# yangt1013/SPEINet

Hardware: AMD Instinct MI355X
Metric: deblurred 720p frames/sec (higher is better)
Workload: dtype f16 (correlation top2)

## Files before the change

### speinet_amd/csrc/conv64_ws16.hip

```cpp
#include "common.h"

namespace {

constexpr int C = 64, KS = 5, PAD = 2, NTAP = KS * KS;
constexpr int TH = 6, TW = 32;
constexpr int IH = TH + KS - 1, IW = TW + KS - 1;
constexpr int PITCH = 2 * C + 16;
constexpr int SLAB = IH * IW * PITCH;
constexpr int NTHR = 256;
constexpr int HR = TH / 2;
constexpr int XCH_WAVE = HR * 4 * 64 * 16;
constexpr int LDS_BYTES = 2 * SLAB + 4 * XCH_WAVE;
constexpr int PF = 1;

struct WsParams {
    const void* a;
    const void* wfrag;
    const float* bias;
    void* out;
    int H, W, batch, act;
    int tiles_x, tiles_y, total;
    long long* stamps;
};

__device__ __forceinline__ void mfma_aw(f32x16& acc, const lpv<_Float16>::x8& w, const lpv<_Float16>::x8& b) {
    asm volatile("v_mfma_f32_32x32x16_f16 %0, %1, %2, %0" : "+v"(acc) : "a"(w), "v"(b));
}
__device__ __forceinline__ void mfma_aw(f32x16& acc, const lpv<__bf16>::x8& w, const lpv<__bf16>::x8& b) {
    asm volatile("v_mfma_f32_32x32x16_bf16 %0, %1, %2, %0" : "+v"(acc) : "a"(w), "v"(b));
}
__device__ __forceinline__ void mfma_aw0(f32x16& acc, const lpv<_Float16>::x8& w, const lpv<_Float16>::x8& b) {
    asm volatile("v_mfma_f32_32x32x16_f16 %0, %1, %2, 0" : "=v"(acc) : "a"(w), "v"(b));
}
__device__ __forceinline__ void mfma_aw0(f32x16& acc, const lpv<__bf16>::x8& w, const lpv<__bf16>::x8& b) {
    asm volatile("v_mfma_f32_32x32x16_bf16 %0, %1, %2, 0" : "=v"(acc) : "a"(w), "v"(b));
}

template <typename TA> struct Chunk { static constexpr int CPP = sizeof(TA) == 4 ? 16 : 8; };

template <typename LP, typename TA, typename TO>
__global__ __launch_bounds__(NTHR, 1) void conv64_ws_kernel(const WsParams p) {
    typedef typename lpv<LP>::x8 lp8;
    typedef typename lpv<LP>::x4 lp4;
    constexpr int CPP = Chunk<TA>::CPP;
    constexpr int NCH = IH * IW * CPP;
    constexpr int NIT = (NCH + NTHR - 1) / NTHR;
    constexpr int NPH = sizeof(TA) == 4 ? 3 : 1;
    constexpr int NITH = (NIT + NPH - 1) / NPH;
    constexpr int PSTEP = 2 * NTAP / NPH;
    static_assert(NPH == 1 || NPH == 3, "the MFMA loop below is cut for one or three staging parts");
    extern __shared__ __attribute__((aligned(16))) unsigned char smem[];

    const int tid = threadIdx.x, lane = tid & 63, wave = tid >> 6;
    const int fr = lane & 31, fk = lane >> 5;
    const int nt = wave >> 1, kh = wave & 1;

    lp8 wreg[NTAP][2];
    {
        const LP* wp = static_cast<const LP*>(p.wfrag) + ((size_t)nt * NTAP * 4 + 2 * kh) * 512 + lane * 8;
#pragma unroll
        for (int t = 0; t < NTAP; ++t)
#pragma unroll
            for (int s = 0; s < 2; ++s) wreg[t][s] = *reinterpret_cast<const lp8*>(wp + (t * 4 + s) * 512);
    }
    float biasv[16];
#pragma unroll
    for (int r = 0; r < 16; ++r) biasv[r] = p.bias ? p.bias[32 * nt + 8 * (r >> 2) + 4 * fk + (r & 3)] : 0.f;

    typedef u32x4 stage_t;
    stage_t sreg[NITH];
    const size_t map_elems = (size_t)p.H * p.W * C;
    const int per_map = p.tiles_x * p.tiles_y;
    const int G = gridDim.x;
    const int slot = (G & 7) ? (int)blockIdx.x : (int)(blockIdx.x & 7) * (G >> 3) + (int)(blockIdx.x >> 3);
    auto tile_of = [&](int t) {
        const int base = t - (int)blockIdx.x;
        return base + G <= p.total ? base + slot : t;
    };
    auto tile_origin = [&](int t, int& b, int& oy0, int& ox0) {
        t = tile_of(t);
        b = t / per_map;
        const int r = t - b * per_map;
        const int ty = r / p.tiles_x;
        oy0 = ty * TH;
        ox0 = (r - ty * p.tiles_x) * TW;
    };
    constexpr int PPI = NTHR / CPP, E = 16 / (int)sizeof(TA);
    const int p0 = tid / CPP, sub = tid - p0 * CPP;
    const int iy0 = p0 / IW, ix0 = p0 - iy0 * IW;
    const int lds0 = p0 * PITCH + sub * (sizeof(TA) == 4 ? 8 : 16);
    auto advance = [](int& iy, int& ix) {
        ix += PPI % IW;
        iy += PPI / IW;
        if (ix >= IW) { ix -= IW; ++iy; }
    };
    auto load_slab = [&](int t, int ph) {
        int b, oy0, ox0;
        tile_origin(t, b, oy0, ox0);
        const TA* base = static_cast<const TA*>(p.a) + (size_t)b * map_elems + sub * E;
        int iy = iy0, ix = ix0;
#pragma unroll
        for (int it = 0; it < NIT; ++it) {
            if (it >= ph * NITH && it < (ph + 1) * NITH) {
                const int iyc = min(iy, IH - 1);
                const int gy = min(max(oy0 - PAD + iyc, 0), p.H - 1), gx = min(max(ox0 - PAD + ix, 0), p.W - 1);
                sreg[it - ph * NITH] = *reinterpret_cast<const stage_t*>(base + ((size_t)gy * p.W + gx) * C);
            }
            advance(iy, ix);
        }
    };
    auto store_slab = [&](int t, int buf, int ph, int lo, int hi) {
        int b, oy0, ox0;
        tile_origin(t, b, oy0, ox0);
        unsigned char* sl = smem + buf * SLAB + lds0;
        int iy = iy0, ix = ix0;
#pragma unroll
        for (int it = 0; it < NIT; ++it) {
            if (it >= ph * NITH + lo && it < ph * NITH + hi && it < (ph + 1) * NITH && iy < IH) {
                const int j = it - ph * NITH;
                const bool ok = ((unsigned)(oy0 - PAD + iy) < (unsigned)p.H) & ((unsigned)(ox0 - PAD + ix) < (unsigned)p.W);
                if constexpr (sizeof(TA) == 4) {
                    const f32x4 v = __builtin_bit_cast(f32x4, sreg[j]);
                    lp4 h = to_lp4<LP>(v);
                    if (!ok) h = lp4{(LP)0.f, (LP)0.f, (LP)0.f, (LP)0.f};
                    *reinterpret_cast<lp4*>(sl + it * PPI * PITCH) = h;
                } else {
                    *reinterpret_cast<stage_t*>(sl + it * PPI * PITCH) = ok ? sreg[j] : stage_t{0u, 0u, 0u, 0u};
                }
            }
            advance(iy, ix);
        }
    };

    int t = blockIdx.x;
    if (t >= p.total) return;
#pragma unroll
    for (int ph = 0; ph < NPH; ++ph) {
        load_slab(t, ph);
        store_slab(t, 0, ph, 0, NITH);
    }
    lds_barrier();

    int boff[TH];
#pragma unroll
    for (int i = 0; i < TH; ++i) boff[i] = (((i + HR * kh) % TH) * IW + fr) * PITCH + kh * 64 + fk * 16;
    unsigned char* const xch = smem + 2 * SLAB;

    int buf = 0;
    for (; t < p.total; t += gridDim.x, buf ^= 1) {
        const int tn = t + gridDim.x;
        const bool more = tn < p.total;
        const int tl = more ? tn : t;
        const bool st_ = t == (int)blockIdx.x + (int)gridDim.x;
        if (st_) SPEI_STAMP(p.stamps, 0);
        load_slab(tl, 0);
        if (st_) SPEI_STAMP(p.stamps, 1);
        __builtin_amdgcn_sched_barrier(0);

        const unsigned char* sl = smem + buf * SLAB;
        f32x16 acc[TH];
        lp8 bq[PF + 1][TH];
        auto step_off = [](int step) { const int tap = step >> 1; return ((tap / KS) * IW + (tap % KS)) * PITCH + (step & 1) * 32; };
#pragma unroll
        for (int d = 0; d < PF; ++d)
#pragma unroll
            for (int i = 0; i < TH; ++i) bq[d][i] = *reinterpret_cast<const lp8*>(sl + boff[i] + step_off(d));
        auto steps = [&](auto lo_c, auto hi_c) {
            constexpr int LO = decltype(lo_c)::value, HI = decltype(hi_c)::value;
#pragma unroll
            for (int step = LO; step < HI; ++step) {
                const int tap = step >> 1, s2 = step & 1;
                if (step + PF < NTAP * 2) {
#pragma unroll
                    for (int i = 0; i < TH; ++i)
                        bq[(step + PF) % (PF + 1)][i] = *reinterpret_cast<const lp8*>(sl + boff[i] + step_off(step + PF));
                }
#pragma unroll
                for (int i = 0; i < TH; ++i) {
                    if (step == 0) mfma_aw0(acc[i], wreg[tap][s2], bq[step % (PF + 1)][i]);
                    else mfma_aw(acc[i], wreg[tap][s2], bq[step % (PF + 1)][i]);
                }
                if (NPH == 1 && step >= NTAP && ((step - NTAP) & 1) == 0 && (step - NTAP) / 2 < NITH)
                    store_slab(tl, buf ^ 1, 0, (step - NTAP) / 2, (step - NTAP) / 2 + 1);
            }
        };
        if constexpr (NPH == 1) {
            steps(std::integral_constant<int, 0>{}, std::integral_constant<int, 2 * NTAP>{});
        } else {
            steps(std::integral_constant<int, 0>{}, std::integral_constant<int, PSTEP>{});
            store_slab(tl, buf ^ 1, 0, 0, NITH);
            load_slab(tl, 1);
            steps(std::integral_constant<int, PSTEP>{}, std::integral_constant<int, 2 * PSTEP>{});
            store_slab(tl, buf ^ 1, 1, 0, NITH);
            load_slab(tl, 2);
            steps(std::integral_constant<int, 2 * PSTEP>{}, std::integral_constant<int, 2 * NTAP>{});
        }

        __builtin_amdgcn_sched_barrier(0);
        asm volatile("s_nop 7\n\ts_nop 7\n\ts_nop 7" ::: "memory");
        __builtin_amdgcn_sched_barrier(0);
        if (st_) SPEI_STAMP(p.stamps, 2);
        {
            f32x4* x = reinterpret_cast<f32x4*>(xch + wave * XCH_WAVE) + lane;
#pragma unroll
            for (int j = 0; j < HR; ++j)
#pragma unroll
                for (int g = 0; g < 4; ++g)
                    x[(j * 4 + g) * 64] = f32x4{acc[HR + j][4 * g], acc[HR + j][4 * g + 1], acc[HR + j][4 * g + 2], acc[HR + j][4 * g + 3]};
        }
        lds_barrier();
        if (st_) SPEI_STAMP(p.stamps, 3);
        {
            int b, oy0, ox0;
            tile_origin(t, b, oy0, ox0);
            TO* ob = static_cast<TO*>(p.out) + (size_t)b * map_elems;
            const int ox = ox0 + fr;
            const f32x4* x = reinterpret_cast<const f32x4*>(xch + (wave ^ 1) * XCH_WAVE) + lane;
#pragma unroll
            for (int j = 0; j < HR; ++j) {
                const int oy = oy0 + kh * HR + j;
                if (oy < p.H && ox < p.W) {
                    TO* o = ob + ((size_t)oy * p.W + ox) * C + 32 * nt + 4 * fk;
#pragma unroll
                    for (int g = 0; g < 4; ++g) {
                        const f32x4 q = x[(j * 4 + g) * 64];
                        f32x4 v;
#pragma unroll
                        for (int e = 0; e < 4; ++e) {
                            v[e] = acc[j][4 * g + e] + q[e] + biasv[4 * g + e];
                            if (p.act == SPEI_ACT_RELU) v[e] = fmaxf(v[e], 0.f);
                        }
                        if constexpr (sizeof(TO) == 4) *reinterpret_cast<f32x4*>(o + 8 * g) = v;
                        else *reinterpret_cast<lp4*>(o + 8 * g) = to_lp4<LP>(v);
                    }
                }
            }
        }
        if (st_) SPEI_STAMP(p.stamps, 4);
        if (NPH > 1) store_slab(tl, buf ^ 1, NPH - 1, 0, NITH);
        else store_slab(tl, buf ^ 1, 0, (NTAP + 1) / 2, NITH);
        lds_barrier();
        if (st_) SPEI_STAMP(p.stamps, 5);
    }
}

template <typename LP>
int launch_ws(const WsParams& p, int a16, int o16, hipStream_t st) {
    const size_t lds = LDS_BYTES;
    const int cus = spei_num_cus();
    const dim3 grid(p.total < cus ? p.total : cus);
    if (a16 && o16) {
        ensure_dyn_lds<&conv64_ws_kernel<LP, LP, LP>>(lds);
        hipLaunchKernelGGL((conv64_ws_kernel<LP, LP, LP>), grid, dim3(NTHR), lds, st, p);
    } else if (!a16 && o16) {
        ensure_dyn_lds<&conv64_ws_kernel<LP, float, LP>>(lds);
        hipLaunchKernelGGL((conv64_ws_kernel<LP, float, LP>), grid, dim3(NTHR), lds, st, p);
    } else if (a16 && !o16) {
        ensure_dyn_lds<&conv64_ws_kernel<LP, LP, float>>(lds);
        hipLaunchKernelGGL((conv64_ws_kernel<LP, LP, float>), grid, dim3(NTHR), lds, st, p);
    } else {
        ensure_dyn_lds<&conv64_ws_kernel<LP, float, float>>(lds);
        hipLaunchKernelGGL((conv64_ws_kernel<LP, float, float>), grid, dim3(NTHR), lds, st, p);
    }
    return 0;
}

}

extern "C" int spei_conv64_ws16(int fmt, const void* a, int a_fmt, const void* wfrag, const float* bias, void* out, int out_fmt, int batch,
                                int H, int W, int act, spei_stream_t stream) {
    SPEI_REQUIRE(a && wfrag && out, "spei_conv64_ws16: null pointer");
    SPEI_REQUIRE((fmt == SPEI_BF16 || fmt == SPEI_F16) && (a_fmt == SPEI_F32 || a_fmt == fmt) && (out_fmt == SPEI_F32 || out_fmt == fmt),
                 "spei_conv64_ws16: fmt=%d a_fmt=%d out_fmt=%d", fmt, a_fmt, out_fmt);
    SPEI_REQUIRE(batch >= 1 && H > 0 && W > 0 && (int64_t)batch * cdiv(H, TH) * cdiv(W, TW) < (1ll << 30) && (int64_t)H * W < (1ll << 26),
                 "spei_conv64_ws16: batch=%d of %dx%d", batch, H, W);
    SPEI_REQUIRE(act == SPEI_ACT_NONE || act == SPEI_ACT_RELU, "spei_conv64_ws16: act=%d", act);
    SPEI_REQUIRE(((uintptr_t)a | (uintptr_t)wfrag | (uintptr_t)out) % 16 == 0 && a != out, "spei_conv64_ws16: 16-byte alignment, out must not be the input");
    WsParams p;
    p.a = a; p.wfrag = wfrag; p.bias = bias; p.out = out; p.H = H; p.W = W; p.batch = batch; p.act = act;
    p.tiles_x = cdiv(W, TW); p.tiles_y = cdiv(H, TH); p.total = batch * p.tiles_x * p.tiles_y;
    p.stamps = spei_stamp_buffer();
    hipStream_t st = (hipStream_t)stream;
    const int a16 = a_fmt != SPEI_F32, o16 = out_fmt != SPEI_F32;
    const int rc = fmt == SPEI_F16 ? launch_ws<_Float16>(p, a16, o16, st) : launch_ws<__bf16>(p, a16, o16, st);
    if (rc) return rc;
    SPEI_CHECK_LAUNCH("spei_conv64_ws16");
    return 0;
}
```

### speinet_amd/csrc/resblock.hip

```cpp
#include "common.h"

namespace {

constexpr int GATE_TR16 = 16;
constexpr int GATE_TR32 = 8;
__host__ __device__ inline int gate_tr(bool lp) { return lp ? GATE_TR16 : GATE_TR32; }
__host__ __device__ inline int gate_tc(int C) { return 256 / (C / 8); }

struct GateWs {
    float* rowpmax;
    float* rowpsum;
    float* colpmax;
    float* colpsum;
    float* tilesum;
    int ntx, nty;
};
__host__ __device__ inline GateWs carve(float* ws, int H, int W, int C, bool lp) {
    GateWs g;
    g.ntx = (W + gate_tc(C) - 1) / gate_tc(C);
    g.nty = (H + gate_tr(lp) - 1) / gate_tr(lp);
    g.rowpmax = ws;
    g.rowpsum = g.rowpmax + (size_t)g.ntx * H * C;
    g.colpmax = g.rowpsum + (size_t)g.ntx * H * C;
    g.colpsum = g.colpmax + (size_t)g.nty * W * C;
    g.tilesum = g.colpsum + (size_t)g.nty * W * C;
    return g;
}

template <typename T>
__device__ __forceinline__ f32x4 ld4(const T* p) {
    if constexpr (sizeof(T) == 4) {
        return *reinterpret_cast<const f32x4*>(p);
    } else {
        const typename lpv<T>::x4 h = *reinterpret_cast<const typename lpv<T>::x4*>(p);
        return f32x4{(float)h[0], (float)h[1], (float)h[2], (float)h[3]};
    }
}

__device__ __forceinline__ f32x4 max4(f32x4 a, f32x4 b) {
    return f32x4{fmaxf(a[0], b[0]), fmaxf(a[1], b[1]), fmaxf(a[2], b[2]), fmaxf(a[3], b[3])};
}

template <int C, typename TX>
__global__ __launch_bounds__(256) void gate_stats_kernel(const TX* __restrict__ x1, int H, int W, float* ws, int64_t wsf) {
    constexpr bool LP = sizeof(TX) == 2;
    x1 += (size_t)blockIdx.y * H * W * C;
    const GateWs g = carve(ws + (size_t)blockIdx.y * wsf, H, W, C, LP);
    constexpr int OCT = C / 8;
    constexpr int TC = 256 / OCT;
    constexpr int TR = LP ? GATE_TR16 : GATE_TR32;
    constexpr int EB = LP ? 16 : 32;
    constexpr int ROWB = TC * OCT * EB + 4 * EB;
    constexpr int ITEMS = TR * OCT;
    constexpr int PARTS = 256 / ITEMS;
    constexpr int SEG = TC / PARTS;
    extern __shared__ __attribute__((aligned(16))) unsigned char tile[];
    float* rsum = reinterpret_cast<float*>(tile + TR * ROWB);
    const int tid = threadIdx.x;
    const int oct = tid % OCT, col = tid / OCT;
    const int tx = blockIdx.x % g.ntx, ty = blockIdx.x / g.ntx;
    const int x = tx * TC + col, y0 = ty * TR;

    u32x4 v[TR][LP ? 1 : 2];
#pragma unroll
    for (int r = 0; r < TR; ++r) {
        const bool ok = x < W && y0 + r < H;
        const TX* src = x1 + ((size_t)min(y0 + r, H - 1) * W + min(x, W - 1)) * C + oct * 8;
#pragma unroll
        for (int hlf = 0; hlf < (LP ? 1 : 2); ++hlf) {
            v[r][hlf] = *reinterpret_cast<const u32x4*>(reinterpret_cast<const unsigned char*>(src) + 16 * hlf);
            if (!ok) v[r][hlf] = u32x4{0u, 0u, 0u, 0u};
        }
    }
    auto unpack = [](const u32x4* q, float* f) __attribute__((always_inline)) {
        if constexpr (LP) {
            const typename lpv<TX>::x8 h = *reinterpret_cast<const typename lpv<TX>::x8*>(q);
#pragma unroll
            for (int e = 0; e < 8; ++e) f[e] = (float)h[e];
        } else {
#pragma unroll
            for (int e = 0; e < 8; ++e) f[e] = __uint_as_float(q[e >> 2][e & 3]);
        }
    };
    float cmax[8], csum[8];
#pragma unroll
    for (int e = 0; e < 8; ++e) { cmax[e] = -INFINITY; csum[e] = 0.f; }
#pragma unroll
    for (int r = 0; r < TR; ++r) {
        float f[8];
        unpack(v[r], f);
        if (y0 + r < H) {
#pragma unroll
            for (int e = 0; e < 8; ++e) { cmax[e] = fmaxf(cmax[e], f[e]); csum[e] += f[e]; }
        }
#pragma unroll
        for (int hlf = 0; hlf < (LP ? 1 : 2); ++hlf)
            *reinterpret_cast<u32x4*>(tile + r * ROWB + (col * OCT + oct) * EB + 16 * hlf) = v[r][hlf];
    }
    if (x < W) {
        float* pm = g.colpmax + ((size_t)ty * W + x) * C + oct * 8;
        float* ps = g.colpsum + ((size_t)ty * W + x) * C + oct * 8;
        *reinterpret_cast<f32x4*>(pm) = f32x4{cmax[0], cmax[1], cmax[2], cmax[3]};
        *reinterpret_cast<f32x4*>(pm + 4) = f32x4{cmax[4], cmax[5], cmax[6], cmax[7]};
        *reinterpret_cast<f32x4*>(ps) = f32x4{csum[0], csum[1], csum[2], csum[3]};
        *reinterpret_cast<f32x4*>(ps + 4) = f32x4{csum[4], csum[5], csum[6], csum[7]};
    }
    __syncthreads();

    {
        const int part = tid % PARTS, item = tid / PARTS;
        const int ro = item % OCT, rr = item / OCT;
        float rmax[8], rs[8];
#pragma unroll
        for (int e = 0; e < 8; ++e) { rmax[e] = -INFINITY; rs[e] = 0.f; }
        const int ncol = min(TC, W - tx * TC);
#pragma unroll 4
        for (int j = 0; j < SEG; ++j) {
            const int c2 = j * PARTS + part;
            u32x4 q[LP ? 1 : 2];
#pragma unroll
            for (int hlf = 0; hlf < (LP ? 1 : 2); ++hlf) q[hlf] = *reinterpret_cast<const u32x4*>(tile + rr * ROWB + (c2 * OCT + ro) * EB + 16 * hlf);
            float f[8];
            unpack(q, f);
            if (c2 < ncol) {
#pragma unroll
                for (int e = 0; e < 8; ++e) { rmax[e] = fmaxf(rmax[e], f[e]); rs[e] += f[e]; }
            }
        }
#pragma unroll
        for (int e = 0; e < 8; ++e) {
            if constexpr (PARTS >= 2) { rmax[e] = fmaxf(rmax[e], dpp_quad<0xB1>(rmax[e])); rs[e] += dpp_quad<0xB1>(rs[e]); }
            if constexpr (PARTS >= 4) { rmax[e] = fmaxf(rmax[e], dpp_quad<0x4E>(rmax[e])); rs[e] += dpp_quad<0x4E>(rs[e]); }
            if constexpr (PARTS >= 8) { rmax[e] = fmaxf(rmax[e], dpp_quad<0x141>(rmax[e])); rs[e] += dpp_quad<0x141>(rs[e]); }
        }
        const int y = y0 + rr;
        if (part == 0) {
#pragma unroll
            for (int e = 0; e < 8; ++e) rsum[rr * C + ro * 8 + e] = (y < H) ? rs[e] : 0.f;
            if (y < H) {
                float* pm = g.rowpmax + ((size_t)tx * H + y) * C + ro * 8;
                float* ps = g.rowpsum + ((size_t)tx * H + y) * C + ro * 8;
                *reinterpret_cast<f32x4*>(pm) = f32x4{rmax[0], rmax[1], rmax[2], rmax[3]};
                *reinterpret_cast<f32x4*>(pm + 4) = f32x4{rmax[4], rmax[5], rmax[6], rmax[7]};
                *reinterpret_cast<f32x4*>(ps) = f32x4{rs[0], rs[1], rs[2], rs[3]};
                *reinterpret_cast<f32x4*>(ps + 4) = f32x4{rs[4], rs[5], rs[6], rs[7]};
            }
        }
    }
    __syncthreads();
    if (tid < C) {
        float t = 0.f;
#pragma unroll
        for (int r = 0; r < TR; ++r) t += rsum[r * C + tid];
        g.tilesum[(size_t)blockIdx.x * C + tid] = t;
    }
}

template <int C, typename TX>
void launch_gate_stats(const TX* x1, int H, int W, const GateWs& g, float* ws, int64_t wsf, int batch, hipStream_t st) {
    constexpr bool LP = sizeof(TX) == 2;
    constexpr int OCT = C / 8, TC = 256 / OCT, TR = LP ? GATE_TR16 : GATE_TR32, EB = LP ? 16 : 32;
    const size_t lds = (size_t)TR * (TC * OCT * EB + 4 * EB) + (size_t)TR * C * sizeof(float);
    ensure_dyn_lds<&gate_stats_kernel<C, TX>>(lds);
    hipLaunchKernelGGL((gate_stats_kernel<C, TX>), dim3(g.ntx * g.nty, batch), dim3(256), lds, st, x1, H, W, ws, wsf);
}

__device__ __forceinline__ void reduce_partials(const float* __restrict__ pmax, const float* __restrict__ psum, int nt, int64_t stride,
                                                int l0, int cnt, int L, int C, float, float denom, float* zmax, float* zmean) {
    float mx[4], sm[4];
    int64_t off[4];
    bool ok[4];
#pragma unroll
    for (int j = 0; j < 4; ++j) {
        const int it = threadIdx.x + 256 * j;
        const int line = l0 + it / C;
        ok[j] = it < cnt * C && line >= 0 && line < L;
        off[j] = ok[j] ? (int64_t)line * C + it % C : 0;
        mx[j] = -INFINITY;
        sm[j] = 0.f;
    }
    int k = 0;
    for (; k + 4 <= nt; k += 4) {
        float a[4][4], b[4][4];
#pragma unroll
        for (int u = 0; u < 4; ++u)
#pragma unroll
            for (int j = 0; j < 4; ++j) {
                a[u][j] = pmax[(size_t)(k + u) * stride + off[j]];
                b[u][j] = psum[(size_t)(k + u) * stride + off[j]];
            }
#pragma unroll
        for (int u = 0; u < 4; ++u)
#pragma unroll
            for (int j = 0; j < 4; ++j) { mx[j] = fmaxf(mx[j], a[u][j]); sm[j] += b[u][j]; }
    }
    for (; k < nt; ++k) {
#pragma unroll
        for (int j = 0; j < 4; ++j) {
            const float a = pmax[(size_t)k * stride + off[j]], b = psum[(size_t)k * stride + off[j]];
            mx[j] = fmaxf(mx[j], a);
            sm[j] += b;
        }
    }
#pragma unroll
    for (int j = 0; j < 4; ++j) {
        const int it = threadIdx.x + 256 * j;
        if (it < cnt * C) {
            zmax[it] = ok[j] ? mx[j] : -INFINITY;
            zmean[it] = ok[j] ? sm[j] / denom : 0.f;
        }
    }
}

__global__ __launch_bounds__(256) void gate_maps_kernel(int H, int W, int C, float* ws, int64_t wsf, int lp, const float* __restrict__ cw_w,
                                                        const float* __restrict__ cw_bn, const float* __restrict__ hc_w,
                                                        const float* __restrict__ hc_bn, float* __restrict__ g1,
                                                        float* __restrict__ g2, const float* __restrict__ w1,
                                                        const float* __restrict__ b1, const float* __restrict__ w2,
                                                        const float* __restrict__ b2, float* __restrict__ s) {
    const GateWs g = carve(ws + (size_t)blockIdx.y * wsf, H, W, C, lp != 0);
    g1 += (size_t)blockIdx.y * H * C;
    g2 += (size_t)blockIdx.y * W * C;
    s += (size_t)blockIdx.y * C;
    __shared__ float wk[98];
    __shared__ float zmax[1024], zmean[1024];
    const int64_t n1 = (int64_t)H * C;
    const int nb1 = (int)((n1 + 255) / 256);
    const int nb2 = (int)(((int64_t)W * C + 255) / 256);
    if ((int)blockIdx.x == nb1 + nb2) {
        __shared__ f32x4 part[256];
        __shared__ float mean[128], hid[32];
        const int ntiles = g.ntx * g.nty, cq = C / 4, parts = 256 / cq;
        const int q = threadIdx.x % cq, pt = threadIdx.x / cq;
        const f32x4* ts = reinterpret_cast<const f32x4*>(g.tilesum) + q;
        f32x4 acc[8];
#pragma unroll
        for (int u = 0; u < 8; ++u) acc[u] = f32x4{0.f, 0.f, 0.f, 0.f};
        int t = pt;
        for (; t + 7 * parts < ntiles; t += 8 * parts) {
#pragma unroll
            for (int u = 0; u < 8; ++u) acc[u] += ts[(size_t)(t + u * parts) * cq];
        }
        for (; t < ntiles; t += parts) acc[0] += ts[(size_t)t * cq];
        part[threadIdx.x] = ((acc[0] + acc[1]) + (acc[2] + acc[3])) + ((acc[4] + acc[5]) + (acc[6] + acc[7]));
        __syncthreads();
        if ((int)threadIdx.x < C) {
            const int c = threadIdx.x;
            float a = 0.f;
            for (int k = 0; k < parts; ++k) a += part[k * cq + (c >> 2)][c & 3];
            mean[c] = a / ((float)H * (float)W);
        }
        __syncthreads();
        const int mid = C / 4;
        if ((int)threadIdx.x < mid) {
            float a = b1[threadIdx.x];
            for (int k = 0; k < C; ++k) a = fmaf(w1[threadIdx.x * C + k], mean[k], a);
            hid[threadIdx.x] = fmaxf(a, 0.f);
        }
        __syncthreads();
        if ((int)threadIdx.x < C) {
            float a = b2[threadIdx.x];
            for (int k = 0; k < mid; ++k) a = fmaf(w2[threadIdx.x * mid + k], hid[k], a);
            s[threadIdx.x] = 1.0f / (1.0f + expf(-a));
        }
        return;
    }
    if ((int)blockIdx.x < nb1) {
        if (threadIdx.x < 98) wk[threadIdx.x] = cw_w[threadIdx.x];
        const int64_t i0 = (int64_t)blockIdx.x * 256;
        const int y0 = (int)(i0 / C) - 3, rows = 256 / C + 6;
        reduce_partials(g.rowpmax, g.rowpsum, g.ntx, n1, y0, rows, H, C, 1.0f, (float)W, zmax, zmean);
        __syncthreads();
        const int64_t i = i0 + threadIdx.x;
        if (i >= n1) return;
        const int c = (int)(i % C), y = (int)(i / C);
        float acc = 0.f;
#pragma unroll
        for (int ch = 0; ch < 2; ++ch) {
            const float* z = ch == 0 ? zmax : zmean;
            for (int dy = 0; dy < 7; ++dy) {
                const int yy = y + dy - 3;
                if (yy < 0 || yy >= H) continue;
                for (int dc = 0; dc < 7; ++dc) {
                    const int cc = c + dc - 3;
                    if (cc < 0 || cc >= C) continue;
                    acc = fmaf(wk[ch * 49 + dy * 7 + dc], z[(yy - y0) * C + cc], acc);
                }
            }
        }
        g1[i] = fmaf(acc, cw_bn[0], cw_bn[1]);
    } else {
        if (threadIdx.x < 50) wk[threadIdx.x] = hc_w[threadIdx.x];
        const int64_t n2 = (int64_t)W * C;
        const int64_t i0 = (int64_t)(blockIdx.x - nb1) * 256;
        const int x0 = (int)(i0 / C) - 2, cols = 256 / C + 4;
        reduce_partials(g.colpmax, g.colpsum, g.nty, n2, x0, cols, W, C, 1.0f, (float)H, zmax, zmean);
        __syncthreads();
        const int64_t i = i0 + threadIdx.x;
        if (i >= n2) return;
        const int c = (int)(i % C), x = (int)(i / C);
        float acc = 0.f;
#pragma unroll
        for (int ch = 0; ch < 2; ++ch) {
            const float* z = ch == 0 ? zmax : zmean;
            for (int dc = 0; dc < 5; ++dc) {
                const int cc = c + dc - 2;
                if (cc < 0 || cc >= C) continue;
                for (int dx = 0; dx < 5; ++dx) {
                    const int xx = x + dx - 2;
                    if (xx < 0 || xx >= W) continue;
                    acc = fmaf(wk[ch * 25 + dc * 5 + dx], z[(xx - x0) * C + cc], acc);
                }
            }
        }
        g2[i] = fmaf(acc, hc_bn[0], hc_bn[1]);
    }
}

template <typename T>
__global__ __launch_bounds__(256) void resblock_apply_kernel(const float* __restrict__ x, const T* __restrict__ x1,
                                                             const float* __restrict__ s, const float* __restrict__ g1,
                                                             const float* __restrict__ g2, const float* __restrict__ extra,
                                                             float* __restrict__ out, int ldo, int H, int W, int C) {
    const int cg = C / 4;
    const int64_t total = (int64_t)H * W * cg;
    {
        const size_t b = blockIdx.y;
        x += b * H * W * C; x1 += b * H * W * C; out += b * H * W * ldo;
        s += b * C; g1 += b * H * C; g2 += b * W * C;
    }
    for (int64_t i = (int64_t)blockIdx.x * 256 + threadIdx.x; i < total; i += (int64_t)gridDim.x * 256) {
        const int c = (int)(i % cg) * 4;
        const int64_t pix = i / cg;
        const int xx = (int)(pix % W), yy = (int)(pix / W);
        const float4 a = *reinterpret_cast<const float4*>(x + pix * C + c);
        const f32x4 bv = ld4<T>(x1 + pix * C + c);
        const float4 b = make_float4(bv[0], bv[1], bv[2], bv[3]);
        const float4 sv = *reinterpret_cast<const float4*>(s + c);
        const float4 u = *reinterpret_cast<const float4*>(g1 + (size_t)yy * C + c);
        const float4 v = *reinterpret_cast<const float4*>(g2 + (size_t)xx * C + c);
        float4 o;
        o.x = (b.x * sv.x + (b.x * u.x + b.x * v.x)) + a.x;
        o.y = (b.y * sv.y + (b.y * u.y + b.y * v.y)) + a.y;
        o.z = (b.z * sv.z + (b.z * u.z + b.z * v.z)) + a.z;
        o.w = (b.w * sv.w + (b.w * u.w + b.w * v.w)) + a.w;
        if (extra) {
            const float4 e = *reinterpret_cast<const float4*>(extra + pix * C + c);
            o.x += e.x; o.y += e.y; o.z += e.z; o.w += e.w;
        }
        *reinterpret_cast<float4*>(out + pix * ldo + c) = o;
    }
}

}

extern "C" int64_t spei_gate_ws_floats(int H, int W, int C) {
    if (C != 32 && C != 64 && C != 128) return 0;
    const int64_t ntx = (W + gate_tc(C) - 1) / gate_tc(C), nty = (H + GATE_TR32 - 1) / GATE_TR32;
    return 2 * ntx * H * C + 2 * nty * W * C + ntx * nty * C;
}

static int resblock_gates_run(const void* x1, int x1_fmt, int batch, int H, int W, int C, const float* se_w1, const float* se_b1,
                              const float* se_w2, const float* se_b2, const float* cw_w, const float* cw_bn,
                              const float* hc_w, const float* hc_bn, float* s, float* g1, float* g2, float* ws,
                              spei_stream_t stream) {
    SPEI_REQUIRE(batch >= 1 && batch <= 65535, "spei_resblock_gates_batched: batch=%d", batch);
    SPEI_REQUIRE(x1 && se_w1 && se_b1 && se_w2 && se_b2 && cw_w && cw_bn && hc_w && hc_bn && s && g1 && g2 && ws,
                 "spei_resblock_gates: null pointer");
    SPEI_REQUIRE(C == 32 || C == 64 || C == 128, "spei_resblock_gates: C=%d (32/64/128 built)", C);
    SPEI_REQUIRE(H > 0 && W > 0, "spei_resblock_gates: empty map");
    SPEI_REQUIRE(((uintptr_t)x1 | (uintptr_t)ws) % 16 == 0, "spei_resblock_gates: 16-byte alignment required");
    hipStream_t st = (hipStream_t)stream;
    SPEI_REQUIRE(x1_fmt == SPEI_F32 || x1_fmt == SPEI_BF16 || x1_fmt == SPEI_F16, "spei_resblock_gates: x1_fmt=%d", x1_fmt);
    GateWs g = carve(ws, H, W, C, x1_fmt != SPEI_F32);
    const int64_t wsf = spei_gate_ws_floats(H, W, C);
    if (x1_fmt == SPEI_BF16) {
        const __bf16* xp = (const __bf16*)x1;
        if (C == 32) launch_gate_stats<32>(xp, H, W, g, ws, wsf, batch, st);
        else if (C == 64) launch_gate_stats<64>(xp, H, W, g, ws, wsf, batch, st);
        else launch_gate_stats<128>(xp, H, W, g, ws, wsf, batch, st);
    } else if (x1_fmt == SPEI_F16) {
        const _Float16* xp = (const _Float16*)x1;
        if (C == 32) launch_gate_stats<32>(xp, H, W, g, ws, wsf, batch, st);
        else if (C == 64) launch_gate_stats<64>(xp, H, W, g, ws, wsf, batch, st);
        else launch_gate_stats<128>(xp, H, W, g, ws, wsf, batch, st);
    } else {
        const float* xp = (const float*)x1;
        if (C == 32) launch_gate_stats<32>(xp, H, W, g, ws, wsf, batch, st);
        else if (C == 64) launch_gate_stats<64>(xp, H, W, g, ws, wsf, batch, st);
        else launch_gate_stats<128>(xp, H, W, g, ws, wsf, batch, st);
    }
    hipLaunchKernelGGL(gate_maps_kernel, dim3(cdiv((int64_t)H * C, 256) + cdiv((int64_t)W * C, 256) + 1, batch), dim3(256), 0, st, H, W, C, ws, wsf,
                       (int)(x1_fmt != SPEI_F32), cw_w, cw_bn, hc_w, hc_bn, g1, g2, se_w1, se_b1, se_w2, se_b2, s);
    SPEI_CHECK_LAUNCH("spei_resblock_gates");
    return 0;
}

extern "C" int spei_resblock_gates(const void* x1, int x1_fmt, int H, int W, int C, const float* se_w1, const float* se_b1,
                                   const float* se_w2, const float* se_b2, const float* cw_w, const float* cw_bn,
                                   const float* hc_w, const float* hc_bn, float* s, float* g1, float* g2, float* ws,
                                   spei_stream_t stream) {
    return resblock_gates_run(x1, x1_fmt, 1, H, W, C, se_w1, se_b1, se_w2, se_b2, cw_w, cw_bn, hc_w, hc_bn, s, g1, g2, ws, stream);
}

extern "C" int spei_resblock_gates_batched(const void* x1, int x1_fmt, int batch, int H, int W, int C, const float* se_w1, const float* se_b1,
                                           const float* se_w2, const float* se_b2, const float* cw_w, const float* cw_bn,
                                           const float* hc_w, const float* hc_bn, float* s, float* g1, float* g2, float* ws,
                                           spei_stream_t stream) {
    return resblock_gates_run(x1, x1_fmt, batch, H, W, C, se_w1, se_b1, se_w2, se_b2, cw_w, cw_bn, hc_w, hc_bn, s, g1, g2, ws, stream);
}

static int resblock_apply_run(const float* x, const void* x1, int x1_fmt, const float* s, const float* g1, const float* g2,
                              const float* extra, float* out, int ldo, int batch, int H, int W, int C, spei_stream_t stream) {
    SPEI_REQUIRE(x && x1 && s && g1 && g2 && out, "spei_resblock_apply: null pointer");
    SPEI_REQUIRE(batch >= 1 && batch <= 65535 && (batch == 1 || (!extra && ldo == C)), "spei_resblock_apply_batched: dense maps, no `extra`");
    SPEI_REQUIRE(C % 4 == 0 && ldo % 4 == 0 && ldo >= C && H > 0 && W > 0, "spei_resblock_apply: bad shape");
    const int64_t total = (int64_t)H * W * (C / 4);
    const int blocks = (int)((total + 255) / 256 < 8192 ? (total + 255) / 256 : 8192);
    const dim3 grid(blocks, batch);
    SPEI_REQUIRE(x1_fmt == SPEI_F32 || x1_fmt == SPEI_BF16 || x1_fmt == SPEI_F16, "spei_resblock_apply: x1_fmt=%d", x1_fmt);
    if (x1_fmt == SPEI_BF16) hipLaunchKernelGGL(resblock_apply_kernel<__bf16>, grid, dim3(256), 0, (hipStream_t)stream, x, (const __bf16*)x1, s, g1, g2, extra, out, ldo, H, W, C);
    else if (x1_fmt == SPEI_F16) hipLaunchKernelGGL(resblock_apply_kernel<_Float16>, grid, dim3(256), 0, (hipStream_t)stream, x, (const _Float16*)x1, s, g1, g2, extra, out, ldo, H, W, C);
    else hipLaunchKernelGGL(resblock_apply_kernel<float>, grid, dim3(256), 0, (hipStream_t)stream, x, (const float*)x1, s, g1, g2, extra, out, ldo, H, W, C);
    SPEI_CHECK_LAUNCH("spei_resblock_apply");
    return 0;
}

extern "C" int spei_resblock_apply(const float* x, const void* x1, int x1_fmt, const float* s, const float* g1, const float* g2,
                                   const float* extra, float* out, int ldo, int H, int W, int C, spei_stream_t stream) {
    return resblock_apply_run(x, x1, x1_fmt, s, g1, g2, extra, out, ldo, 1, H, W, C, stream);
}

extern "C" int spei_resblock_apply_batched(const float* x, const void* x1, int x1_fmt, const float* s, const float* g1, const float* g2,
                                           float* out, int batch, int H, int W, int C, spei_stream_t stream) {
    return resblock_apply_run(x, x1, x1_fmt, s, g1, g2, nullptr, out, C, batch, H, W, C, stream);
}
```

Before: 40.86.

## Software-pipeline conv epilogue and slab staging into half-step MFMA schedule

The per-tile MFMA loop is split into two halves over row groups, so one half's partial sums are exchanged through LDS while the other half still computes. The epilogue (bias, activation, global store) of the previous tile is interleaved into the next tile's MFMA stream, and the global loads and LDS stores for the next slab are spread chunk by chunk across compile-time half-steps. Prefetch depth rises to two. The aim is to hide the epilogue, the exchange and the staging behind matrix math instead of running them serially. The cost is a hand-tuned schedule tied to specific NITH values, higher register pressure, and a final drain after the loop.

```diff
diff --git a/speinet_amd/csrc/conv64_ws16.hip b/speinet_amd/csrc/conv64_ws16.hip
--- a/speinet_amd/csrc/conv64_ws16.hip
+++ b/speinet_amd/csrc/conv64_ws16.hip
@@ -11,7 +11,10 @@
 constexpr int HR = TH / 2;
 constexpr int XCH_WAVE = HR * 4 * 64 * 16;
 constexpr int LDS_BYTES = 2 * SLAB + 4 * XCH_WAVE;
-constexpr int PF = 1;
+constexpr int NHS = 4 * NTAP;
+constexpr int PF = 2;
+constexpr int FIN0 = 2;
+constexpr int XW0 = NHS / 2 + 2;
 
 struct WsParams {
     const void* a;
@@ -38,6 +41,29 @@
 
 template <typename TA> struct Chunk { static constexpr int CPP = sizeof(TA) == 4 ? 16 : 8; };
 
+template <int I, int N, typename F>
+__device__ __forceinline__ void static_for(F&& f) {
+    if constexpr (I < N) {
+        f(std::integral_constant<int, I>{});
+        static_for<I + 1, N>(f);
+    }
+}
+
+constexpr int ld_chunk(int nph, int hh) {
+    if (nph == 3) return hh / 35 < 3 && hh % 35 < 8 ? 8 * (hh / 35) + hh % 35 : -1;
+    return hh >= NHS / 4 + 1 && hh < NHS / 4 + 25 && (hh - NHS / 4 - 1) % 2 == 0 ? (hh - NHS / 4 - 1) / 2 : -1;
+}
+constexpr int st_chunk(int nph, int hh) {
+    if (nph == 3) {
+        for (int ph = 0; ph < 3; ++ph) {
+            const int s = ph == 2 ? 93 : 27 + 35 * ph;
+            if (hh >= s && hh < s + 8) return 8 * ph + hh - s;
+        }
+        return -1;
+    }
+    return hh >= NHS / 2 + 2 && (hh - NHS / 2 - 2) % 4 == 0 && (hh - NHS / 2 - 2) / 4 < 12 ? (hh - NHS / 2 - 2) / 4 : -1;
+}
+
 template <typename LP, typename TA, typename TO>
 __global__ __launch_bounds__(NTHR, 1) void conv64_ws_kernel(const WsParams p) {
     typedef typename lpv<LP>::x8 lp8;
@@ -47,8 +73,7 @@
     constexpr int NIT = (NCH + NTHR - 1) / NTHR;
     constexpr int NPH = sizeof(TA) == 4 ? 3 : 1;
     constexpr int NITH = (NIT + NPH - 1) / NPH;
-    constexpr int PSTEP = 2 * NTAP / NPH;
-    static_assert(NPH == 1 || NPH == 3, "the MFMA loop below is cut for one or three staging parts");
+    static_assert((NPH == 1 && NITH == 12) || (NPH == 3 && NITH == 8), "ld_chunk / st_chunk are cut for these two schedules");
     extern __shared__ __attribute__((aligned(16))) unsigned char smem[];
 
     const int tid = threadIdx.x, lane = tid & 63, wave = tid >> 6;
@@ -94,14 +119,14 @@
         iy += PPI / IW;
         if (ix >= IW) { ix -= IW; ++iy; }
     };
-    auto load_slab = [&](int t, int ph) {
+    auto load_slab = [&](int t, int ph, int lo, int hi) {
         int b, oy0, ox0;
         tile_origin(t, b, oy0, ox0);
         const TA* base = static_cast<const TA*>(p.a) + (size_t)b * map_elems + sub * E;
         int iy = iy0, ix = ix0;
 #pragma unroll
         for (int it = 0; it < NIT; ++it) {
-            if (it >= ph * NITH && it < (ph + 1) * NITH) {
+            if (it >= ph * NITH + lo && it < ph * NITH + hi && it < (ph + 1) * NITH) {
                 const int iyc = min(iy, IH - 1);
                 const int gy = min(max(oy0 - PAD + iyc, 0), p.H - 1), gx = min(max(ox0 - PAD + ix, 0), p.W - 1);
                 sreg[it - ph * NITH] = *reinterpret_cast<const stage_t*>(base + ((size_t)gy * p.W + gx) * C);
@@ -136,7 +161,7 @@
     if (t >= p.total) return;
 #pragma unroll
     for (int ph = 0; ph < NPH; ++ph) {
-        load_slab(t, ph);
+        load_slab(t, ph, 0, NITH);
         store_slab(t, 0, ph, 0, NITH);
     }
     lds_barrier();
@@ -145,6 +170,37 @@
 #pragma unroll
     for (int i = 0; i < TH; ++i) boff[i] = (((i + HR * kh) % TH) * IW + fr) * PITCH + kh * 64 + fk * 16;
     unsigned char* const xch = smem + 2 * SLAB;
+    f32x4* const xw = reinterpret_cast<f32x4*>(xch + wave * XCH_WAVE) + lane;
+    const f32x4* const xr = reinterpret_cast<const f32x4*>(xch + (wave ^ 1) * XCH_WAVE) + lane;
+    auto frag_off = [&](int hh, int i) {
+        const int step = hh % (NHS / 2), tap = step >> 1;
+        return boff[(hh < NHS / 2 ? HR : 0) + i] + ((tap / KS) * IW + (tap % KS)) * PITCH + (step & 1) * 32;
+    };
+
+    f32x16 acc[TH];
+#pragma unroll
+    for (int i = 0; i < HR; ++i)
+#pragma unroll
+        for (int r = 0; r < 16; ++r) acc[i][r] = 0.f;
+
+    int fb = 0, foy0 = p.H, fox0 = 0;
+    f32x4 q;
+    auto fin_read = [&](int k) { q = xr[k * 64]; };
+    auto fin_store = [&](int k) {
+        const int j = k >> 2, g = k & 3;
+        const int oy = foy0 + kh * HR + j, ox = fox0 + fr;
+        if (oy < p.H && ox < p.W) {
+            TO* o = static_cast<TO*>(p.out) + (size_t)fb * map_elems + ((size_t)oy * p.W + ox) * C + 32 * nt + 4 * fk;
+            f32x4 v;
+#pragma unroll
+            for (int e = 0; e < 4; ++e) {
+                v[e] = acc[j][4 * g + e] + q[e] + biasv[4 * g + e];
+                if (p.act == SPEI_ACT_RELU) v[e] = fmaxf(v[e], 0.f);
+            }
+            if constexpr (sizeof(TO) == 4) *reinterpret_cast<f32x4*>(o + 8 * g) = v;
+            else *reinterpret_cast<lp4*>(o + 8 * g) = to_lp4<LP>(v);
+        }
+    };
 
     int buf = 0;
     for (; t < p.total; t += gridDim.x, buf ^= 1) {
@@ -153,94 +209,58 @@
         const int tl = more ? tn : t;
         const bool st_ = t == (int)blockIdx.x + (int)gridDim.x;
         if (st_) SPEI_STAMP(p.stamps, 0);
-        load_slab(tl, 0);
+        const unsigned char* sl = smem + buf * SLAB;
+        lp8 bq[PF + 1][HR];
+#pragma unroll
+        for (int d = 0; d < PF; ++d)
+#pragma unroll
+            for (int i = 0; i < HR; ++i) bq[d][i] = *reinterpret_cast<const lp8*>(sl + frag_off(d, i));
         if (st_) SPEI_STAMP(p.stamps, 1);
         __builtin_amdgcn_sched_barrier(0);
 
-        const unsigned char* sl = smem + buf * SLAB;
-        f32x16 acc[TH];
-        lp8 bq[PF + 1][TH];
-        auto step_off = [](int step) { const int tap = step >> 1; return ((tap / KS) * IW + (tap % KS)) * PITCH + (step & 1) * 32; };
-#pragma unroll
-        for (int d = 0; d < PF; ++d)
-#pragma unroll
-            for (int i = 0; i < TH; ++i) bq[d][i] = *reinterpret_cast<const lp8*>(sl + boff[i] + step_off(d));
-        auto steps = [&](auto lo_c, auto hi_c) {
-            constexpr int LO = decltype(lo_c)::value, HI = decltype(hi_c)::value;
-#pragma unroll
-            for (int step = LO; step < HI; ++step) {
-                const int tap = step >> 1, s2 = step & 1;
-                if (step + PF < NTAP * 2) {
-#pragma unroll
-                    for (int i = 0; i < TH; ++i)
-                        bq[(step + PF) % (PF + 1)][i] = *reinterpret_cast<const lp8*>(sl + boff[i] + step_off(step + PF));
-                }
-#pragma unroll
-                for (int i = 0; i < TH; ++i) {
-                    if (step == 0) mfma_aw0(acc[i], wreg[tap][s2], bq[step % (PF + 1)][i]);
-                    else mfma_aw(acc[i], wreg[tap][s2], bq[step % (PF + 1)][i]);
-                }
-                if (NPH == 1 && step >= NTAP && ((step - NTAP) & 1) == 0 && (step - NTAP) / 2 < NITH)
-                    store_slab(tl, buf ^ 1, 0, (step - NTAP) / 2, (step - NTAP) / 2 + 1);
-            }
+        auto halfstep = [&](auto hc) {
+            constexpr int hh = decltype(hc)::value;
+            constexpr int step = hh % (NHS / 2), tap = step >> 1, s2 = step & 1, a0 = hh < NHS / 2 ? HR : 0;
+            if constexpr (hh + PF < NHS) {
+#pragma unroll
+                for (int i = 0; i < HR; ++i) bq[(hh + PF) % (PF + 1)][i] = *reinterpret_cast<const lp8*>(sl + frag_off(hh + PF, i));
+            }
+#pragma unroll
+            for (int i = 0; i < HR; ++i) {
+                if constexpr (step == 0) mfma_aw0(acc[a0 + i], wreg[tap][s2], bq[hh % (PF + 1)][i]);
+                else mfma_aw(acc[a0 + i], wreg[tap][s2], bq[hh % (PF + 1)][i]);
+            }
+            if constexpr (hh >= FIN0 && hh < FIN0 + 2 * HR * 4) {
+                if constexpr (((hh - FIN0) & 1) == 0) fin_read((hh - FIN0) >> 1);
+                else fin_store((hh - FIN0) >> 1);
+            }
+            if constexpr (hh >= XW0 && hh < XW0 + HR * 4) {
+                constexpr int k = hh - XW0, j = k >> 2, g = k & 3;
+                xw[k * 64] = f32x4{acc[HR + j][4 * g], acc[HR + j][4 * g + 1], acc[HR + j][4 * g + 2], acc[HR + j][4 * g + 3]};
+            }
+            constexpr int lc = ld_chunk(NPH, hh), sc = st_chunk(NPH, hh);
+            if constexpr (lc >= 0) load_slab(tl, lc / NITH, lc % NITH, lc % NITH + 1);
+            if constexpr (sc >= 0) store_slab(tl, buf ^ 1, sc / NITH, sc % NITH, sc % NITH + 1);
+            __builtin_amdgcn_sched_barrier(0);
         };
-        if constexpr (NPH == 1) {
-            steps(std::integral_constant<int, 0>{}, std::integral_constant<int, 2 * NTAP>{});
-        } else {
-            steps(std::integral_constant<int, 0>{}, std::integral_constant<int, PSTEP>{});
-            store_slab(tl, buf ^ 1, 0, 0, NITH);
-            load_slab(tl, 1);
-            steps(std::integral_constant<int, PSTEP>{}, std::integral_constant<int, 2 * PSTEP>{});
-            store_slab(tl, buf ^ 1, 1, 0, NITH);
-            load_slab(tl, 2);
-            steps(std::integral_constant<int, 2 * PSTEP>{}, std::integral_constant<int, 2 * NTAP>{});
-        }
-
-        __builtin_amdgcn_sched_barrier(0);
-        asm volatile("s_nop 7\n\ts_nop 7\n\ts_nop 7" ::: "memory");
-        __builtin_amdgcn_sched_barrier(0);
+        static_for<0, NHS / 2>(halfstep);
         if (st_) SPEI_STAMP(p.stamps, 2);
-        {
-            f32x4* x = reinterpret_cast<f32x4*>(xch + wave * XCH_WAVE) + lane;
-#pragma unroll
-            for (int j = 0; j < HR; ++j)
-#pragma unroll
-                for (int g = 0; g < 4; ++g)
-                    x[(j * 4 + g) * 64] = f32x4{acc[HR + j][4 * g], acc[HR + j][4 * g + 1], acc[HR + j][4 * g + 2], acc[HR + j][4 * g + 3]};
-        }
         lds_barrier();
         if (st_) SPEI_STAMP(p.stamps, 3);
-        {
-            int b, oy0, ox0;
-            tile_origin(t, b, oy0, ox0);
-            TO* ob = static_cast<TO*>(p.out) + (size_t)b * map_elems;
-            const int ox = ox0 + fr;
-            const f32x4* x = reinterpret_cast<const f32x4*>(xch + (wave ^ 1) * XCH_WAVE) + lane;
-#pragma unroll
-            for (int j = 0; j < HR; ++j) {
-                const int oy = oy0 + kh * HR + j;
-                if (oy < p.H && ox < p.W) {
-                    TO* o = ob + ((size_t)oy * p.W + ox) * C + 32 * nt + 4 * fk;
-#pragma unroll
-                    for (int g = 0; g < 4; ++g) {
-                        const f32x4 q = x[(j * 4 + g) * 64];
-                        f32x4 v;
-#pragma unroll
-                        for (int e = 0; e < 4; ++e) {
-                            v[e] = acc[j][4 * g + e] + q[e] + biasv[4 * g + e];
-                            if (p.act == SPEI_ACT_RELU) v[e] = fmaxf(v[e], 0.f);
-                        }
-                        if constexpr (sizeof(TO) == 4) *reinterpret_cast<f32x4*>(o + 8 * g) = v;
-                        else *reinterpret_cast<lp4*>(o + 8 * g) = to_lp4<LP>(v);
-                    }
-                }
-            }
-        }
+        static_for<NHS / 2, NHS>(halfstep);
         if (st_) SPEI_STAMP(p.stamps, 4);
-        if (NPH > 1) store_slab(tl, buf ^ 1, NPH - 1, 0, NITH);
-        else store_slab(tl, buf ^ 1, 0, (NTAP + 1) / 2, NITH);
+        tile_origin(t, fb, foy0, fox0);
         lds_barrier();
         if (st_) SPEI_STAMP(p.stamps, 5);
+    }
+
+    __builtin_amdgcn_sched_barrier(0);
+    asm volatile("s_nop 7\n\ts_nop 7\n\ts_nop 7" ::: "memory");
+    __builtin_amdgcn_sched_barrier(0);
+#pragma unroll
+    for (int k = 0; k < HR * 4; ++k) {
+        fin_read(k);
+        fin_store(k);
     }
 }
 
```

New measurement: 41.05, median of 6. No clear change (+0.5%).

## Make gate stats blocks loop over multi-tile row segments with prefetch

Applied to the files above, without the earlier changes.

The gate statistics kernel now has each block walk a vertical segment of several row tiles instead of a single tile, with the segment length chosen so that roughly a minimum number of blocks is launched. Column partials are accumulated across the whole segment, which shrinks the column-partial and tile-sum buffers and the reduction work in the later gate kernel. The next tile's global loads are issued after the LDS barrier so they overlap with the row reduction. In exchange there is less block-level parallelism and an extra barrier per iteration, and the workspace size now depends on the segment calculation.

```diff
diff --git a/speinet_amd/csrc/resblock.hip b/speinet_amd/csrc/resblock.hip
--- a/speinet_amd/csrc/resblock.hip
+++ b/speinet_amd/csrc/resblock.hip
@@ -4,8 +4,14 @@
 
 constexpr int GATE_TR16 = 16;
 constexpr int GATE_TR32 = 8;
+constexpr int GATE_MIN_BLOCKS = 256;
 __host__ __device__ inline int gate_tr(bool lp) { return lp ? GATE_TR16 : GATE_TR32; }
 __host__ __device__ inline int gate_tc(int C) { return 256 / (C / 8); }
+__host__ __device__ inline int gate_seg_rows(int H, int W, int C, bool lp) {
+    const int ntx = (W + gate_tc(C) - 1) / gate_tc(C), nty = (H + gate_tr(lp) - 1) / gate_tr(lp);
+    const int k = (int)((int64_t)ntx * nty / GATE_MIN_BLOCKS);
+    return (k < 1 ? 1 : k) * gate_tr(lp);
+}
 
 struct GateWs {
     float* rowpmax;
@@ -13,17 +19,18 @@
     float* colpmax;
     float* colpsum;
     float* tilesum;
-    int ntx, nty;
+    int ntx, nseg, segr;
 };
 __host__ __device__ inline GateWs carve(float* ws, int H, int W, int C, bool lp) {
     GateWs g;
     g.ntx = (W + gate_tc(C) - 1) / gate_tc(C);
-    g.nty = (H + gate_tr(lp) - 1) / gate_tr(lp);
+    g.segr = gate_seg_rows(H, W, C, lp);
+    g.nseg = (H + g.segr - 1) / g.segr;
     g.rowpmax = ws;
     g.rowpsum = g.rowpmax + (size_t)g.ntx * H * C;
     g.colpmax = g.rowpsum + (size_t)g.ntx * H * C;
-    g.colpsum = g.colpmax + (size_t)g.nty * W * C;
-    g.tilesum = g.colpsum + (size_t)g.nty * W * C;
+    g.colpsum = g.colpmax + (size_t)g.nseg * W * C;
+    g.tilesum = g.colpsum + (size_t)g.nseg * W * C;
     return g;
 }
 
@@ -49,7 +56,8 @@
     constexpr int OCT = C / 8;
     constexpr int TC = 256 / OCT;
     constexpr int TR = LP ? GATE_TR16 : GATE_TR32;
-    constexpr int EB = LP ? 16 : 32;
+    constexpr int NV = LP ? 1 : 2;
+    constexpr int EB = 16 * NV;
     constexpr int ROWB = TC * OCT * EB + 4 * EB;
     constexpr int ITEMS = TR * OCT;
     constexpr int PARTS = 256 / ITEMS;
@@ -58,20 +66,21 @@
     float* rsum = reinterpret_cast<float*>(tile + TR * ROWB);
     const int tid = threadIdx.x;
     const int oct = tid % OCT, col = tid / OCT;
-    const int tx = blockIdx.x % g.ntx, ty = blockIdx.x / g.ntx;
-    const int x = tx * TC + col, y0 = ty * TR;
-
-    u32x4 v[TR][LP ? 1 : 2];
-#pragma unroll
-    for (int r = 0; r < TR; ++r) {
-        const bool ok = x < W && y0 + r < H;
-        const TX* src = x1 + ((size_t)min(y0 + r, H - 1) * W + min(x, W - 1)) * C + oct * 8;
-#pragma unroll
-        for (int hlf = 0; hlf < (LP ? 1 : 2); ++hlf) {
-            v[r][hlf] = *reinterpret_cast<const u32x4*>(reinterpret_cast<const unsigned char*>(src) + 16 * hlf);
-            if (!ok) v[r][hlf] = u32x4{0u, 0u, 0u, 0u};
-        }
-    }
+    const int tx = blockIdx.x % g.ntx, sg = blockIdx.x / g.ntx;
+    const int x = tx * TC + col;
+    const int ybeg = sg * g.segr, yend = min(H, ybeg + g.segr);
+    const int ncol = min(TC, W - tx * TC);
+
+    const TX* colbase = x1 + (size_t)min(x, W - 1) * C + oct * 8;
+    u32x4 v[TR][NV];
+    auto load = [&](int y0) __attribute__((always_inline)) {
+#pragma unroll
+        for (int r = 0; r < TR; ++r) {
+            const unsigned char* src = reinterpret_cast<const unsigned char*>(colbase + (size_t)min(y0 + r, H - 1) * W * C);
+#pragma unroll
+            for (int hlf = 0; hlf < NV; ++hlf) v[r][hlf] = *reinterpret_cast<const u32x4*>(src + 16 * hlf);
+        }
+    };
     auto unpack = [](const u32x4* q, float* f) __attribute__((always_inline)) {
         if constexpr (LP) {
             const typename lpv<TX>::x8 h = *reinterpret_cast<const typename lpv<TX>::x8*>(q);
@@ -85,41 +94,36 @@
     float cmax[8], csum[8];
 #pragma unroll
     for (int e = 0; e < 8; ++e) { cmax[e] = -INFINITY; csum[e] = 0.f; }
-#pragma unroll
-    for (int r = 0; r < TR; ++r) {
-        float f[8];
-        unpack(v[r], f);
-        if (y0 + r < H) {
-#pragma unroll
-            for (int e = 0; e < 8; ++e) { cmax[e] = fmaxf(cmax[e], f[e]); csum[e] += f[e]; }
-        }
-#pragma unroll
-        for (int hlf = 0; hlf < (LP ? 1 : 2); ++hlf)
-            *reinterpret_cast<u32x4*>(tile + r * ROWB + (col * OCT + oct) * EB + 16 * hlf) = v[r][hlf];
-    }
-    if (x < W) {
-        float* pm = g.colpmax + ((size_t)ty * W + x) * C + oct * 8;
-        float* ps = g.colpsum + ((size_t)ty * W + x) * C + oct * 8;
-        *reinterpret_cast<f32x4*>(pm) = f32x4{cmax[0], cmax[1], cmax[2], cmax[3]};
-        *reinterpret_cast<f32x4*>(pm + 4) = f32x4{cmax[4], cmax[5], cmax[6], cmax[7]};
-        *reinterpret_cast<f32x4*>(ps) = f32x4{csum[0], csum[1], csum[2], csum[3]};
-        *reinterpret_cast<f32x4*>(ps + 4) = f32x4{csum[4], csum[5], csum[6], csum[7]};
-    }
-    __syncthreads();
-
-    {
-        const int part = tid % PARTS, item = tid / PARTS;
-        const int ro = item % OCT, rr = item / OCT;
+    float tsum = 0.f;
+    const int part = tid % PARTS, item = tid / PARTS;
+    const int ro = item % OCT, rr = item / OCT;
+
+    load(ybeg);
+    for (int y0 = ybeg; y0 < yend; y0 += TR) {
+#pragma unroll
+        for (int r = 0; r < TR; ++r) {
+            float f[8];
+            unpack(v[r], f);
+            if (y0 + r < H) {
+#pragma unroll
+                for (int e = 0; e < 8; ++e) { cmax[e] = fmaxf(cmax[e], f[e]); csum[e] += f[e]; }
+            }
+#pragma unroll
+            for (int hlf = 0; hlf < NV; ++hlf)
+                *reinterpret_cast<u32x4*>(tile + r * ROWB + (col * OCT + oct) * EB + 16 * hlf) = v[r][hlf];
+        }
+        __syncthreads();
+        if (y0 + TR < yend) load(y0 + TR);
+
         float rmax[8], rs[8];
 #pragma unroll
         for (int e = 0; e < 8; ++e) { rmax[e] = -INFINITY; rs[e] = 0.f; }
-        const int ncol = min(TC, W - tx * TC);
 #pragma unroll 4
         for (int j = 0; j < SEG; ++j) {
             const int c2 = j * PARTS + part;
-            u32x4 q[LP ? 1 : 2];
-#pragma unroll
-            for (int hlf = 0; hlf < (LP ? 1 : 2); ++hlf) q[hlf] = *reinterpret_cast<const u32x4*>(tile + rr * ROWB + (c2 * OCT + ro) * EB + 16 * hlf);
+            u32x4 q[NV];
+#pragma unroll
+            for (int hlf = 0; hlf < NV; ++hlf) q[hlf] = *reinterpret_cast<const u32x4*>(tile + rr * ROWB + (c2 * OCT + ro) * EB + 16 * hlf);
             float f[8];
             unpack(q, f);
             if (c2 < ncol) {
@@ -146,14 +150,21 @@
                 *reinterpret_cast<f32x4*>(ps + 4) = f32x4{rs[4], rs[5], rs[6], rs[7]};
             }
         }
-    }
-    __syncthreads();
-    if (tid < C) {
-        float t = 0.f;
-#pragma unroll
-        for (int r = 0; r < TR; ++r) t += rsum[r * C + tid];
-        g.tilesum[(size_t)blockIdx.x * C + tid] = t;
-    }
+        __syncthreads();
+        if (tid < C) {
+#pragma unroll
+            for (int r = 0; r < TR; ++r) tsum += rsum[r * C + tid];
+        }
+    }
+    if (x < W) {
+        float* pm = g.colpmax + ((size_t)sg * W + x) * C + oct * 8;
+        float* ps = g.colpsum + ((size_t)sg * W + x) * C + oct * 8;
+        *reinterpret_cast<f32x4*>(pm) = f32x4{cmax[0], cmax[1], cmax[2], cmax[3]};
+        *reinterpret_cast<f32x4*>(pm + 4) = f32x4{cmax[4], cmax[5], cmax[6], cmax[7]};
+        *reinterpret_cast<f32x4*>(ps) = f32x4{csum[0], csum[1], csum[2], csum[3]};
+        *reinterpret_cast<f32x4*>(ps + 4) = f32x4{csum[4], csum[5], csum[6], csum[7]};
+    }
+    if (tid < C) g.tilesum[(size_t)blockIdx.x * C + tid] = tsum;
 }
 
 template <int C, typename TX>
@@ -162,7 +173,7 @@
     constexpr int OCT = C / 8, TC = 256 / OCT, TR = LP ? GATE_TR16 : GATE_TR32, EB = LP ? 16 : 32;
     const size_t lds = (size_t)TR * (TC * OCT * EB + 4 * EB) + (size_t)TR * C * sizeof(float);
     ensure_dyn_lds<&gate_stats_kernel<C, TX>>(lds);
-    hipLaunchKernelGGL((gate_stats_kernel<C, TX>), dim3(g.ntx * g.nty, batch), dim3(256), lds, st, x1, H, W, ws, wsf);
+    hipLaunchKernelGGL((gate_stats_kernel<C, TX>), dim3(g.ntx * g.nseg, batch), dim3(256), lds, st, x1, H, W, ws, wsf);
 }
 
 __device__ __forceinline__ void reduce_partials(const float* __restrict__ pmax, const float* __restrict__ psum, int nt, int64_t stride,
@@ -230,7 +241,7 @@
     if ((int)blockIdx.x == nb1 + nb2) {
         __shared__ f32x4 part[256];
         __shared__ float mean[128], hid[32];
-        const int ntiles = g.ntx * g.nty, cq = C / 4, parts = 256 / cq;
+        const int ntiles = g.ntx * g.nseg, cq = C / 4, parts = 256 / cq;
         const int q = threadIdx.x % cq, pt = threadIdx.x / cq;
         const f32x4* ts = reinterpret_cast<const f32x4*>(g.tilesum) + q;
         f32x4 acc[8];
@@ -294,7 +305,7 @@
         const int64_t n2 = (int64_t)W * C;
         const int64_t i0 = (int64_t)(blockIdx.x - nb1) * 256;
         const int x0 = (int)(i0 / C) - 2, cols = 256 / C + 4;
-        reduce_partials(g.colpmax, g.colpsum, g.nty, n2, x0, cols, W, C, 1.0f, (float)H, zmax, zmean);
+        reduce_partials(g.colpmax, g.colpsum, g.nseg, n2, x0, cols, W, C, 1.0f, (float)H, zmax, zmean);
         __syncthreads();
         const int64_t i = i0 + threadIdx.x;
         if (i >= n2) return;
@@ -356,8 +367,11 @@
 
 extern "C" int64_t spei_gate_ws_floats(int H, int W, int C) {
     if (C != 32 && C != 64 && C != 128) return 0;
-    const int64_t ntx = (W + gate_tc(C) - 1) / gate_tc(C), nty = (H + GATE_TR32 - 1) / GATE_TR32;
-    return 2 * ntx * H * C + 2 * nty * W * C + ntx * nty * C;
+    const int64_t ntx = (W + gate_tc(C) - 1) / gate_tc(C);
+    const int r16 = gate_seg_rows(H, W, C, true), r32 = gate_seg_rows(H, W, C, false);
+    const int64_t n16 = (H + r16 - 1) / r16, n32 = (H + r32 - 1) / r32;
+    const int64_t nseg = n16 > n32 ? n16 : n32;
+    return 2 * ntx * H * C + 2 * nseg * W * C + ntx * nseg * C;
 }
 
 static int resblock_gates_run(const void* x1, int x1_fmt, int batch, int H, int W, int C, const float* se_w1, const float* se_b1,
```

Result: no change. 41.19 before, 41.28 after, median of 6 (+0.2%).
